# alenxav/bWGR

Measured on AMD Instinct MI355X. Metric: MCMC iter/sec (full marker sweep), higher is better.
Workload: dtype f32 scalars, fixed-point / f64 residual, int8 genotypes; 1 GPU; c4: synthetic n=10000 x p=1000000 int8, BayesB pi=0.99 (1.2% of the markers in the model at the last sweep), exact chain (blocked sweep, block=128, 40 slabs x 256 rows + 1 sequencer, the chain alone on the GPU: 80 streamers x 128 rows, engine generation 3, lag 12 blocks); n=10000, p=1000000, model=BayesB, df=5, chains=1

## Files before the change

bwgr_amd/csrc/sweep3.hip.h:

```cpp
#pragma once
#include "sweep2.hip.h"

namespace bwgr {

#ifdef BWGR_STAMPS
#define S3ST_DECL unsigned long long ph3[8] = {0, 0, 0, 0, 0, 0, 0, 0}, tl3 = __builtin_amdgcn_s_memtime()
#define S3ST(k, cond) do { if ((BWGR_STAMPS == 1 || (BWGR_STAMPS == 2 && ((k) == 0 || (k) == 1 || (k) == 4)) || (BWGR_STAMPS == 3 && ((k) == 0 || (k) == 4) && blockIdx.x == 0 && threadIdx.x == 0) || (BWGR_STAMPS == 4 && (k) <= 5 && blockIdx.x == 0 && threadIdx.x == 0)) && (cond)) { const unsigned long long t_ = __builtin_amdgcn_s_memtime(); ph3[k] += t_ - tl3; tl3 = t_; } } while (0)
#define S3ST_FLUSH(base, cond) do { if ((cond) && a.stamps) for (int k_ = 0; k_ < 8; ++k_) atomicAdd(&a.stamps[(base) + k_], ph3[k_]); } while (0)
#else
#define S3ST_DECL do { } while (0)
#define S3ST(k, cond) do { } while (0)
#define S3ST_FLUSH(base, cond) do { } while (0)
#endif

static constexpr int S3_MAXD = 16;
static constexpr int S3_LSTRIDE = 2 * SW_MAXM + 2;
static constexpr int S3_ND = 7;
static constexpr int S3_RING = S3_MAXD * SW_MAXM;
static constexpr int S3_GPD_BYTES = 16384;
static constexpr int S3_ROWSLOT = 1024;
static constexpr int S3_NRX = 8;
static constexpr int S3_OS = 12;
static constexpr int S3_NFW = 4;
static constexpr int S3_NFL = 8;
// ... 477 lines not shown
#undef S3_COMMIT1
#undef S3_TILE_COMMIT
}

template <int R3, int NTB, typename SH = S3ShapeAny>
__device__ __forceinline__ void s3_streamer_dma(const Sweep3Args &A) {
#ifdef BWGR_EXPERIMENTS
  const int SDBG = A.dbg;
#else
  constexpr int SDBG = 0;
#endif
  extern __shared__ __attribute__((aligned(16))) unsigned char smem[];
  const SweepArgs &a = A.a;
  const int tid = threadIdx.x, lane = tid & 63, wave = tid >> 6;
  const int m16 = lane & 15, grp = lane >> 4;
  const int w = s3_stream_index(A);
  const unsigned long long *lists_w = A.lists;
  const int m = s3_m<SH>(a), R = a.R, D = A.D;
  constexpr int Rp = R3 + 16;
  constexpr int CH = R3 / 16;
  constexpr int MPP = 1024 / R3;
  constexpr int NPC = SW_MAXM / MPP;
  static_assert(R3 == 128 || R3 == 256, "sixteen or thirty-two pieces");
  const int slab = w / A.sub, hsub = w - slab * A.sub;
  const int nb = a.blk_end - a.blk_begin;
  constexpr int NU = R3 >> 6;
  const int8_t *Xs = reinterpret_cast<const int8_t *>(a.X) + (size_t)slab * a.p * R + (size_t)hsub * R3;
  const int64_t row0 = (int64_t)slab * R + (int64_t)hsub * R3;
  uint32_t *abortw = a.xflags + (size_t)a.K * SW_FLAG_STRIDE;
  constexpr size_t tile_b = (size_t)SW_MAXM * R3;
  int8_t *tile0 = reinterpret_cast<int8_t *>(smem);
  size_t off = NTB * tile_b;
  const uint32_t tile_la = (uint32_t)__builtin_amdgcn_readfirstlane((int)(uint32_t)(uintptr_t)(__attribute__((address_space(3))) const unsigned char *)smem);
  int8_t *edig0 = reinterpret_cast<int8_t *>(smem + off); off += (size_t)2 * 16 * Rp;
  int8_t *ddig0 = reinterpret_cast<int8_t *>(smem + off); off += (size_t)2 * 16 * S2_DP;
  int *outu = reinterpret_cast<int *>(smem + off); off += (size_t)64 * S3_OS * 4 * 4;
  off += (size_t)8 * 32 * S3_OS * 4;
  uint32_t *ctl_s = reinterpret_cast<uint32_t *>(smem + off); off += 64;
  float *drej_s = reinterpret_cast<float *>(smem + off);
  const uint32_t drej_la = (uint32_t)__builtin_amdgcn_readfirstlane((int)(uint32_t)(uintptr_t)(__attribute__((address_space(3))) const unsigned char *)drej_s);
  const int sh = a.sc->e3_sh;
  const double S = s3_pow2(sh), invS = s3_pow2(-sh);
  auto blk_j0 = [&](int b) { return (a.blk_begin + b) * m; };
  auto blk_m = [&](int b) { return min(m, a.p - (a.blk_begin + b) * m); };

  for (int i = tid; i < (int)((2 * 16 * Rp + 2 * 16 * S2_DP) / 4); i += SW_THREADS) reinterpret_cast<uint32_t *>(edig0)[i] = 0u;
  if (tid < 16) ctl_s[tid] = 0u;
  long long e_own = 0;
  const bool upd = wave < NU;
  if (upd) e_own = __double2ll_rn(a.e[row0 + 64 * wave + lane] * S);

  static_assert(NU == 2, "waves 0-1 update, 2-5 dots, 6-7 DMA");
  constexpr int NDOT = 4, PPW = NPC / 2;
  static_assert(NU + NDOT == 6 && SW_THREADS - SW_MAXM == 64 * (NU + NDOT), "the DMA waves (role 2) are the last two: they digitise the rejected steps");
  constexpr int LPS = PPW + 2;
  const uint32_t lane_mk = (uint32_t)(lane / CH), lane_cr = (uint32_t)(lane % CH);
  const int j_lo = a.blk_begin * m, j_hi = min(a.p, a.blk_end * m);
  const int wvs = __builtin_amdgcn_readfirstlane(wave);
  auto drej_issue = [&](int t) {
    const unsigned char *src = reinterpret_cast<const unsigned char *>(a.ps.blocks[a.blk_begin + max(0, min(t, nb - 1))].drej);
    const uint32_t la = drej_la + (uint32_t)((max(t, 0) % NTB) * SW_MAXM * 4);
    s3_dma4s(src, (uint32_t)lane * 4u, la);
    s3_dma4s(src, 256u + (uint32_t)lane * 4u, la + 256u);
  };
  auto tile_issue = [&](int t) {
    if (wvs < 6) return;
    const int jb = blk_j0(min(t, nb - 1));
    const uint32_t la0 = tile_la + (uint32_t)__builtin_amdgcn_readfirstlane((int)((t % NTB) * (int)tile_b));
#pragma unroll
    for (int u = 0; u < PPW; ++u) {
      const int pc = (wvs - 6) + 2 * u;
      const int jl = MPP * pc + (int)lane_mk;
      const int jj = min(jb + jl, j_hi - 1);
      const uint32_t voff = (uint32_t)(jj - j_lo) * (uint32_t)R + ((lane_cr ^ ((uint32_t)jl & (uint32_t)(CH - 1))) * 16u);
      s3_dma16s(reinterpret_cast<const unsigned char *>(Xs + (size_t)j_lo * R), voff, la0 + (uint32_t)pc * 1024u);
    }
    drej_issue(t + 1);
  };

  auto fold_list = [&](int bs, unsigned long long pre, int e_first = 0) -> int {
    const int Bs = a.blk_begin + bs;
    const unsigned long long *L = lists_w + (size_t)Bs * S3_LSTRIDE;
    const int8_t *col = Xs + (size_t)(Bs * m) * R + 64 * wave + lane;
    const uint64_t t0 = wall_clock64();
    unsigned spins = 0;
    unsigned long long hv = __builtin_amdgcn_readfirstlane((uint32_t)pre) | ((unsigned long long)__builtin_amdgcn_readfirstlane((uint32_t)(pre >> 32)) << 32);
    while (!s3_epoch_is(hv, A.epoch)) {
      hv = ld_agent_raw64(L);
      hv = __builtin_amdgcn_readfirstlane((uint32_t)hv) | ((unsigned long long)__builtin_amdgcn_readfirstlane((uint32_t)(hv >> 32)) << 32);
      if (s3_epoch_is(hv, A.epoch)) break;
      if ((++spins & 63u) == 0u) {
        if (ld_agent_u32(abortw) != 0u) return 0;
        if (wall_clock64() - t0 > SW_TIMEOUT_TICKS) { st_agent_u32(abortw, 1u); return 0; }
      }
      __builtin_amdgcn_s_sleep(1);
    }
    const int cnt = (int)(uint32_t)hv;
    for (int c0 = 0; c0 < cnt; c0 += 31) {
      const int nw = min(62, 2 * (cnt - c0));
      unsigned long long wv = pre;
      bool have = (c0 == 0);
      for (;;) {
        const bool mine = lane >= 1 && lane <= nw;
        if (!have) wv = mine ? ld_agent_raw64(L + 2 * c0 + lane) : 0ull;
        if (__ballot(mine && !s3_epoch_is(wv, A.epoch)) == 0ull) break;
        have = false;
        if ((++spins & 63u) == 0u) {
          if (ld_agent_u32(abortw) != 0u) return 0;
          if (wall_clock64() - t0 > SW_TIMEOUT_TICKS) { st_agent_u32(abortw, 1u); return 0; }
        }
        __builtin_amdgcn_s_sleep(1);
      }
      const uint32_t wlo = (uint32_t)wv, whi = (uint32_t)(wv >> 32);
      for (int e0 = (c0 == 0) ? e_first : 0; e0 < nw / 2; e0 += 8) {
        int xb[8]; long long cq[8];
#pragma unroll
        for (int u = 0; u < 8; ++u) {
          const int ee = min(e0 + u, nw / 2 - 1);
          const uint32_t a0 = __builtin_amdgcn_readlane(wlo, 1 + 2 * ee), a1 = __builtin_amdgcn_readlane(whi, 1 + 2 * ee);
          const uint32_t b0 = __builtin_amdgcn_readlane(wlo, 2 + 2 * ee);
          const int k = (int)(a1 & 0xFFu);
          cq[u] = (e0 + u < nw / 2) ? (long long)(((unsigned long long)b0 << 32) | (unsigned long long)a0) : 0ll;
          xb[u] = upd ? (int)col[(size_t)k * R] : 0;
        }
#pragma unroll
        for (int u = 0; u < 8; ++u) e_own -= (long long)xb[u] * cq[u];
      }
    }
    return 1;
  };

  constexpr int NPRE = 4;
  int xp0 = 0, xp1 = 0, xp2 = 0, xp3 = 0;
  long long cp0 = 0, cp1 = 0, cp2 = 0, cp3 = 0;
  int np = -1;
#ifndef BWGR_WORDS2
#define BWGR_WORDS2 0
#endif
  unsigned long long lmid = 0ull, lw1 = 0ull;
#define S3_PAR(A0_, A1_) (*((!BWGR_WORDS2 || PP == 0) ? &(A0_) : &(A1_)))
  auto fold_prefetch = [&](int bs, auto par_c) {
    constexpr int PP = decltype(par_c)::value;
    const unsigned long long wv = S3_PAR(lmid, lw1);
    const unsigned long long hv = __builtin_amdgcn_readfirstlane((uint32_t)wv) | ((unsigned long long)__builtin_amdgcn_readfirstlane((uint32_t)(wv >> 32)) << 32);
    const int cnt = (int)(uint32_t)hv, nw = min(62, 2 * max(cnt, 0));
    const bool ok = bs >= 0 && s3_epoch_is(hv, A.epoch) && __ballot(lane >= 1 && lane <= nw && !s3_epoch_is(wv, A.epoch)) == 0ull;
    const int8_t *col = Xs + (size_t)((a.blk_begin + max(bs, 0)) * m) * R + 64 * wave + lane;
    const uint32_t wlo = (uint32_t)wv, whi = (uint32_t)(wv >> 32);
    const int ne = ok ? nw / 2 : 0;
#define S3_PRE1(U_, XP_, CP_) { \
      const int ee = min(U_, max(ne - 1, 0)); \
      const uint32_t a0 = __builtin_amdgcn_readlane(wlo, 1 + 2 * ee), a1 = __builtin_amdgcn_readlane(whi, 1 + 2 * ee), b0 = __builtin_amdgcn_readlane(wlo, 2 + 2 * ee); \
      CP_ = (U_ < ne) ? (long long)(((unsigned long long)b0 << 32) | (unsigned long long)a0) : 0ll; \
      XP_ = (int)col[(size_t)(ne > 0 ? (int)(a1 & 0xFFu) : 0) * R]; }
    S3_PRE1(0, xp0, cp0) S3_PRE1(1, xp1, cp1) S3_PRE1(2, xp2, cp2) S3_PRE1(3, xp3, cp3)
#undef S3_PRE1
    np = (bs < 0) ? 0 : (ok ? cnt : -1);
  };
  auto fold_pre = [&](int bs) -> int {
#ifdef BWGR_EXPERIMENTS
    if (w == 0 && tid == 0 && a.stamps && (SDBG & (1 << 21))) { atomicAdd(&a.stamps[203], 1ull); if (np < 0) atomicAdd(&a.stamps[202], 1ull); }
#endif
    if (np < 0) return fold_list(bs, 0ull);
    e_own -= (long long)xp0 * cp0 + (long long)xp1 * cp1 + (long long)xp2 * cp2 + (long long)xp3 * cp3;
    return (np > NPRE) ? fold_list(bs, 0ull, NPRE) : 1;
  };

  if (wvs >= 6) drej_issue(0);
  for (int t = 0; t < NTB - 1; ++t) tile_issue(t);
  if (wvs < NU) {
    lmid = ld_agent_raw64(lists_w + (size_t)(a.blk_begin + max(min(1, nb - 1) - D, 0)) * S3_LSTRIDE + lane);
    if (BWGR_WORDS2) lw1 = ld_agent_raw64(lists_w + (size_t)(a.blk_begin + max(min(2, nb - 1) - D, 0)) * S3_LSTRIDE + lane);
  }
  asm volatile("s_waitcnt vmcnt(0)" ::: "memory");
  __syncthreads();
  S3ST_DECL;
  [[maybe_unused]] const bool st_u = (w == 0 && tid == 0), st_d = (w == 0 && tid == 64 * NU);

  constexpr int WN = (NTB - 2) * LPS;
#define S3_DMA_BARRIER() do { if constexpr (DMA) asm volatile("s_waitcnt vmcnt(%0)" : : "n"(WN) : "memory"); asm volatile("s_waitcnt lgkmcnt(0)\n\ts_barrier" ::: "memory"); } while (0)
  auto step = [&](int b, auto par_c, auto role_c) -> bool {
    constexpr int PP = decltype(par_c)::value;
    constexpr int RL = decltype(role_c)::value;
    constexpr bool UPD = RL == 0, DMA = RL == 2;
    const int mB = blk_m(b), par = b & 1;
    S3ST(0, st_u || st_d);
    int8_t *tile = tile0 + (size_t)(b % NTB) * tile_b;
    int8_t *edig = edig0 + (size_t)par * 16 * Rp;
    int8_t *ddig = ddig0 + (size_t)par * 16 * S2_DP;
    if (b >= D && UPD && !(SDBG & 512)) { if (!fold_pre(b - D)) ctl_s[0] = 1u; }
#ifndef BWGR_FOLD_EARLY
#define BWGR_FOLD_EARLY 1
// ... 140 lines not shown
  const int tid = threadIdx.x, lane = tid & 63, wave = tid >> 6;
  static_assert(!SH::fixed || (sizeof(GT) == 2 && !CEN), "the fixed shape: 16-bit Gram entries, columns as stored");
  const int m = s3_m<SH>(a), nb = a.blk_end - a.blk_begin, D = A.D, pstride = s3_pstride<SH>(a);
  size_t off = 0;
  StageBuf *stage = reinterpret_cast<StageBuf *>(smem + off); off += 3 * sizeof(StageBuf);
  double *spec_s = reinterpret_cast<double *>(smem + off); off += (size_t)3 * 2 * SW_MAXM * sizeof(double);
  double *q_s = reinterpret_cast<double *>(smem + off); off += (size_t)2 * SW_MAXM * sizeof(double);
  double *far_s = reinterpret_cast<double *>(smem + off); off += (size_t)2 * S3_NFW * SW_MAXM * sizeof(double);
  float *state_s = reinterpret_cast<float *>(smem + off); off += (size_t)2 * 3 * SW_MAXM * sizeof(float);
  double *accC = reinterpret_cast<double *>(smem + off); off += (size_t)S3_RING * sizeof(double);
  float2 *accS = reinterpret_cast<float2 *>(smem + off); off += (size_t)S3_RING * sizeof(float2);
  int *accK = reinterpret_cast<int *>(smem + off); off += (size_t)S3_RING * sizeof(int);
  unsigned char *rowf_s = smem + off; off += (size_t)2 * S3_NFW * S3_NFL * SW_MAXM * sizeof(GT);
  constexpr bool G16 = (sizeof(GT) == 2);
#ifndef BWGR_GPD3
#define BWGR_GPD3 1
#endif
  constexpr bool GPD = G16 && (BWGR_GPD3 != 0);
  unsigned char *gpd_s = smem + off; if (G16) off += (size_t)3 * S3_GPD_BYTES;
  unsigned char *rowx_s = smem + off; if (G16) off += (size_t)S3_NRX * S3_ROWSLOT;
  unsigned char *qraw_s = smem + off; off += (size_t)3 * S3_QRAW_BYTES;
  unsigned char *touch_s = smem + off; off += 256;
  int *ctrl_s = reinterpret_cast<int *>(smem + off);
  int *pos_s = ctrl_s + 8;
  const unsigned char **gx_s = reinterpret_cast<const unsigned char **>(ctrl_s + 40);
  S3ST_DECL;
  const GT *gp_all = reinterpret_cast<const GT *>(A.gp);
  const float Cc = a.sc->C, odds = a.sc->odds, one_minus_pi = 1.0f - a.sc->pi, Sb = a.sc->Sb;
  const int sh = a.sc->e3_sh;
  const double S = s3_pow2(sh), invS = s3_pow2(-sh);
  uint32_t *abortw = a.xflags + (size_t)a.K * SW_FLAG_STRIDE;
  auto blk_m = [&](int b) { return min(m, a.p - (a.blk_begin + b) * m); };
  auto prow = [&](int k) { return k * (m - 1) - k * (k - 1) / 2; };
  constexpr int NCH = (int)(sizeof(StageBuf) / 16);
  static_assert(NCH + 128 == 512, "four 16-byte chunks for each lane of the two staging waves");

  constexpr int S3_STG_PIECES = 4 + (GPD ? 8 : 0);
  const uint32_t stage_la = (uint32_t)__builtin_amdgcn_readfirstlane((int)(uint32_t)(uintptr_t)(__attribute__((address_space(3))) const unsigned char *)stage);
  const uint32_t spec_la = (uint32_t)__builtin_amdgcn_readfirstlane((int)(uint32_t)(uintptr_t)(__attribute__((address_space(3))) const unsigned char *)spec_s);
  static_assert(sizeof(StageBuf) == 6 * 1024, "six 1 KiB pieces of constants");
  auto stage_issue = [&](int c, int part = -1) {
    const int blk = a.blk_begin + min(c, nb - 1), slot = c % 3, wv2 = __builtin_amdgcn_readfirstlane(wave) - 2;
    const unsigned char *stb = reinterpret_cast<const unsigned char *>(a.ps.blocks + blk);
    const unsigned char *spb = reinterpret_cast<const unsigned char *>(a.ps.spec + blk);
    const uint32_t lo16 = (uint32_t)lane * 16u;
    if (part <= 0) {
#pragma unroll
    for (int u = 0; u < 3; ++u) { const int pc = wv2 + 2 * u; s3_dma16s(stb, (uint32_t)pc * 1024u + lo16, stage_la + (uint32_t)slot * (uint32_t)sizeof(StageBuf) + (uint32_t)pc * 1024u); }
    s3_dma16s(spb, (uint32_t)wv2 * 2048u + lo16, spec_la + (uint32_t)slot * 2048u + (uint32_t)wv2 * 1024u);
    }
    if constexpr (GPD) {
      const int gpbytes = pstride * 2;
      const unsigned char *src = reinterpret_cast<const unsigned char *>(gp_all + (size_t)blk * pstride);
      const uint32_t gla = (uint32_t)__builtin_amdgcn_readfirstlane((int)(uint32_t)(uintptr_t)(__attribute__((address_space(3))) const unsigned char *)gpd_s) + (uint32_t)slot * (uint32_t)S3_GPD_BYTES;
      if (part < 0 || part == 1) {
#pragma unroll
      for (int u = 0; u < 4; ++u) { const int pc = wv2 + 2 * u; s3_dma16s(src, (uint32_t)min(pc * 1024 + lane * 16, gpbytes - 16), gla + (uint32_t)pc * 1024u); }
      }
      if (part < 0 || part == 2) {
#pragma unroll
      for (int u = 4; u < 8; ++u) { const int pc = wv2 + 2 * u; s3_dma16s(src, (uint32_t)min(pc * 1024 + lane * 16, gpbytes - 16), gla + (uint32_t)pc * 1024u); }
      }
    }
  };
#define S3_STG_WAIT() asm volatile("s_waitcnt vmcnt(%0)" : : "n"(S3_STG_PIECES) : "memory")
  const uint32_t qraw_la = (uint32_t)__builtin_amdgcn_readfirstlane((int)(uint32_t)(uintptr_t)(__attribute__((address_space(3))) const unsigned char *)qraw_s);
  const double qweight = (SH::fixed || A.qsplit) ? 4294967296.0 : 16777216.0;
  auto poll_request = [&](int c) {
    const unsigned char *g = reinterpret_cast<const unsigned char *>(A.qsum + (size_t)(a.blk_begin + min(c, nb - 1)) * SW_MAXM * 2);
    const uint32_t la = qraw_la + (uint32_t)((c % 3) * S3_QRAW_BYTES);
    s3_dma16s_sc1(g, (uint32_t)lane * 16u, la);
    s3_dma16s_sc1(g, 1024u + (uint32_t)lane * 16u, la + 1024u);
  };
  auto poll_q = [&](int c) -> int {
    const int mBc = blk_m(c);
    const unsigned long long *g = A.qsum + (size_t)(a.blk_begin + c) * SW_MAXM * 2;
    const unsigned long long need = (unsigned long long)A.K3;
    const bool n0 = lane < mBc, n1 = 64 + lane < mBc;
    asm volatile("s_waitcnt vmcnt(2)" ::: "memory");
    const ulonglong2 v0 = reinterpret_cast<const ulonglong2 *>(qraw_s + (size_t)(c % 3) * S3_QRAW_BYTES)[lane];
    const ulonglong2 v1 = reinterpret_cast<const ulonglong2 *>(qraw_s + (size_t)(c % 3) * S3_QRAW_BYTES)[64 + lane];
    unsigned long long l0 = n0 ? v0.x : need, h0 = n0 ? v0.y : need, l1 = n1 ? v1.x : need, h1 = n1 ? v1.y : need;
    if (__builtin_expect(!(SDBG & 8) && __ballot(!((l0 & 0xFFull) == need && (h0 & 0xFFull) == need && (l1 & 0xFFull) == need && (h1 & 0xFFull) == need)) != 0ull, 0)) {
      const uint64_t t0 = wall_clock64();
      unsigned spins = 0;
#ifdef BWGR_EXPERIMENTS
      if (lane == 0 && a.stamps && (SDBG & (1 << 21))) atomicAdd(&a.stamps[200], 1ull);
#endif
      for (;;) {
        if ((l0 & 0xFFull) == need && (h0 & 0xFFull) == need && (l1 & 0xFFull) == need && (h1 & 0xFFull) == need) break;
        if (SDBG & 8) break;
#ifdef BWGR_EXPERIMENTS
        if (lane == 0 && a.stamps && (SDBG & (1 << 21))) atomicAdd(&a.stamps[201], 1ull);
#endif
        if ((++spins & 63u) == 0u) {
          if (ld_agent_u32(abortw) != 0u) return 0;
          if (wall_clock64() - t0 > SW_TIMEOUT_TICKS) { st_agent_u32(abortw, 1u); return 0; }
        }
        __builtin_amdgcn_s_sleep(1);
        if (n0) { l0 = ld_agent_raw64(g + 2 * lane); h0 = ld_agent_raw64(g + 2 * lane + 1); }
        if (n1) { l1 = ld_agent_raw64(g + 2 * (64 + lane)); h1 = ld_agent_raw64(g + 2 * (64 + lane) + 1); }
      }
    }
    double *qd = q_s + (size_t)(c & 1) * SW_MAXM;
    qd[lane] = n0 ? fma((double)((long long)h0 >> 8), qweight, (double)((long long)l0 >> 8)) * invS : 0.0;
    qd[64 + lane] = n1 ? fma((double)((long long)h1 >> 8), qweight, (double)((long long)l1 >> 8)) * invS : 0.0;
    poll_request(c + 2);
    return 1;
  };
  constexpr int ring = S3_RING;
  static_assert((S3_RING & (S3_RING - 1)) == 0, "ring positions wrap with a mask");
  constexpr int NFL = S3_NFL;
  constexpr int NFW = S3_NFW;
  constexpr int ROWB = SW_MAXM * (int)sizeof(GT);
  constexpr int NPC = ROWB / 256;
  int f_p0 = 0, f_cnt = 0, f_n = 0;
  const uint32_t rowf_la = (uint32_t)__builtin_amdgcn_readfirstlane((int)(uint32_t)(uintptr_t)(__attribute__((address_space(3))) const unsigned char *)rowf_s);
  const int rowbytes = m * (int)sizeof(GT);
  auto far_src = [&](int c, int sl) -> const unsigned char * {
    const int kb = accK[sl];
    const int d = c - (kb >> 8);
    return gx_s[d - 1] + ((size_t)(a.blk_begin + c) * m * m + (size_t)(kb & 0xFF) * m) * sizeof(GT);
  };
  auto far_add = [&](const uint32_t *row, double cf, double &s0, double &s1) {
    if constexpr (sizeof(GT) == 2) { const uint32_t v = row[lane]; s0 = fma((double)(v & 0xFFFFu), cf, s0); s1 = fma((double)(v >> 16), cf, s1); }
    else { s0 = fma((double)(int)row[lane], cf, s0); s1 = fma((double)(int)row[64 + lane], cf, s1); }
  };
  unsigned long long f_ptr = 0ull;
  double f_cf = 0.0;
#ifndef BWGR_FARTOUCH
#define BWGR_FARTOUCH 1
#endif
  auto far_touch = [&](int c) {
    if (!G16 || !BWGR_FARTOUCH || c < 2 || D < 4 || (SDBG & 32)) return;
    const int s_blk = c - 2;
    const int p0 = pos_s[s_blk & 31], cnt = (pos_s[(s_blk + 1) & 31] - p0) & (ring - 1);
    const int q = lane & 31, d = 3 + (q >> 1);
    for (int e0 = 0; e0 < cnt; e0 += 2) {
      const int e = e0 + (lane >> 5);
      if (e < cnt && d <= D - 1 && s_blk + d < nb && (q & 1) * 128 < rowbytes) {
        const int k = accK[(p0 + e) & (ring - 1)] & 0xFF;
        s3_dma4(gx_s[d - 1] + ((size_t)(a.blk_begin + s_blk + d) * m * m + (size_t)k * m) * sizeof(GT) + (size_t)(q & 1) * 128, touch_s);
      }
    }
  };
  int fp_a = 0, fp_b = 0, fp_kb = 0; double fp_cf = 0.0; bool fp_on = false;
  auto far_plan_a = [&](int c) {
    fp_on = !(c < 3 || D < 4 || c >= nb || (SDBG & 32));
    fp_a = pos_s[max(c - D + 1, 0) & 31]; fp_b = pos_s[(max(c, 2) - 2) & 31];
  };
  auto far_plan_b = [&](int c, int hw) {
    f_p0 = fp_a;
    f_cnt = fp_on ? ((fp_b - fp_a) & (ring - 1)) : 0;
    f_n = (f_cnt > hw) ? min(NFL, (f_cnt - hw + NFW - 1) / NFW) : 0;
    const int sl = (f_p0 + hw + NFW * min(lane, max(f_n - 1, 0))) & (ring - 1);
    fp_kb = accK[sl]; fp_cf = accC[sl];
  };
  auto far_plan_c = [&](int c) {
    const int d = min(max(c - (fp_kb >> 8), 1), S3_MAXD);
    const unsigned char *src = gx_s[d - 1] + ((size_t)(a.blk_begin + c) * m * m + (size_t)(fp_kb & 0xFF) * m) * sizeof(GT);
    f_ptr = (f_n > 0) ? (unsigned long long)src : 0ull;
    f_cf = (lane < f_n) ? fp_cf : 0.0;
  };
  auto far_plan = [&](int c, int hw) { far_plan_a(c); far_plan_b(c, hw); far_plan_c(c); };
  auto far_request = [&](int c, int hw) {
    const uint32_t dst_la = (uint32_t)__builtin_amdgcn_readfirstlane((int)(rowf_la + (uint32_t)(((c & 1) * NFW + hw) * NFL) * (uint32_t)ROWB));
    for (int n = 0; n < f_n; ++n) {
      const unsigned char *src = reinterpret_cast<const unsigned char *>(
          (unsigned long long)(uint32_t)__builtin_amdgcn_readlane((int)(uint32_t)f_ptr, n) |
          ((unsigned long long)(uint32_t)__builtin_amdgcn_readlane((int)(uint32_t)(f_ptr >> 32), n) << 32));
#pragma unroll
      for (int pc = 0; pc < NPC; ++pc) s3_dma4s(src, (uint32_t)min(lane * 4 + 256 * pc, rowbytes - 4), dst_la + (uint32_t)(n * ROWB + 256 * pc));
    }
  };
  auto far_consume = [&](int c, int hw, int f_p0, int f_cnt, int f_n, double f_cf) {
    double s0 = 0.0, s1 = 0.0, t0 = 0.0, t1 = 0.0;
    const unsigned char *src = rowf_s + (size_t)(((c & 1) * NFW + hw) * NFL) * ROWB;
    int n = 0;
    if constexpr (sizeof(GT) == 2) {
      for (; n + 4 <= f_n; n += 4) {
// ... 46 lines not shown
  double sum_d = 0.0, sum_b2 = 0.0;
  double chn0 = 1.0, chn1 = 1.0;
  auto chi_request = [&](int c) {
    const StageBuf &sb = a.ps.blocks[a.blk_begin + max(0, min(c, nb - 1))];
    chn0 = sb.chi[lane]; chn1 = sb.chi[64 + lane];
  };
  auto finish_block = [&](int c) {
    const int blk = a.blk_begin + c, j0c = blk * m, mBc = blk_m(c);
    const float *sp = state_s + (size_t)(c & 1) * 2 * SW_MAXM;
    const bool vbv = (a.flags & SWF_VB_VEC) != 0 && !A.skip_vb;
    const double ch0 = chn0, ch1 = chn1;
    if (vbv) chi_request(c + 1);
#pragma unroll
    for (int h = 0; h < 2; ++h) {
      const int t = lane + 64 * h;
      if (t < mBc) {
        const float bn = sp[t], dn = sp[SW_MAXM + t];
        a.b[j0c + t] = bn;
        a.d[j0c + t] = dn;
        if (vbv) a.vb[j0c + t] = (float)((double)(Sb + bn * bn) / (h ? ch1 : ch0));
        sum_d += (double)dn;
        sum_b2 = fma((double)bn, (double)bn, sum_b2);
      }
    }
    const int p0 = pos_s[c & 31], cnt = (pos_s[(c + 1) & 31] - p0) & (ring - 1);
    unsigned long long *L = A.lists + (size_t)blk * S3_LSTRIDE;
    for (int w0 = 0; w0 < 1 + 2 * cnt; w0 += 64) {
      const int wi = w0 + lane;
      if (wi < 1 + 2 * cnt) {
        unsigned long long v;
        if (wi == 0) v = s3_hdr(A.epoch, cnt);
        else {
          const int sl = (p0 + ((wi - 1) >> 1)) & (ring - 1);
          const float2 st2 = accS[sl];
          const long long cq = (long long)rint((double)st2.x * S) - (long long)rint((double)st2.y * S);
          v = ((wi - 1) & 1) ? (((unsigned long long)A.epoch << 40) | (0xEEull << 32) | ((unsigned long long)cq >> 32))
                             : (((unsigned long long)A.epoch << 40) | ((unsigned long long)(uint32_t)(accK[sl] & 0xFF) << 32) | ((unsigned long long)cq & 0xFFFFFFFFull));
        }
        st_agent_raw64(L + wi, v);
      }
    }
  };
#ifndef BWGR_ROLEBAR
#define BWGR_ROLEBAR 1
#endif
#define S3_ROLE_BARRIER() do { if (BWGR_ROLEBAR) asm volatile("s_waitcnt lgkmcnt(0)\n\ts_barrier" ::: "memory"); } while (0)
  const int wvu = __builtin_amdgcn_readfirstlane(wave);

  if (tid < 40) ctrl_s[tid] = (tid == 0) ? 1 : 0;
  if (tid >= 64 && tid < 64 + S3_MAXD) gx_s[tid - 64] = reinterpret_cast<const unsigned char *>(A.gx[tid - 64]);
  __syncthreads();
  if (wave == 1) { poll_request(0); poll_request(1); if (!poll_q(0)) ctrl_s[0] = 0; }
  else if (wave == 2 || wave == 3) { stage_issue(0); stage_issue(1); S3_STG_WAIT(); far_consume(0, wave, 0, 0, 0, 0.0); far_plan(1, wave); far_request(1, wave); }
  else if (wave >= 5 && wave <= 6) { far_consume(0, wave - 5, 0, 0, 0, 0.0); far_plan(1, wave - 5); far_request(1, wave - 5); }
  else if (wave == 7) { for (int c = 0; c < PF; ++c) touch(c); if ((a.flags & SWF_VB_VEC) && !A.skip_vb) chi_request(0); }
  __syncthreads();
  if (ctrl_s[0] == 0) { if (tid == 0) a.sc->error = 1u; asm volatile("s_waitcnt vmcnt(0)" ::: "memory"); return; }
  [[maybe_unused]] const bool sq0 = (tid == 0), sq1 = (tid == 64), sq2 = (tid == 128), sq4 = (tid == 320), sq3 = (tid == 192), sq6 = (tid == 384), sq7 = (tid == 448);
#define S3_BLOCK_END(SQ_, ABORT_) \
    if (!BWGR_ROLEBAR) asm volatile("s_waitcnt lgkmcnt(0)\n\ts_barrier" ::: "memory"); \
    S3ST(4, SQ_); \
    if (ctrl_s[0] == 0) { asm volatile("s_waitcnt vmcnt(0)" ::: "memory"); ABORT_; }
  auto helper_loop = [&](auto &&phase, const bool sq) -> bool {
    for (int b = 0; b < nb; ++b) {
      S3ST(0, sq);
      if (b + 1 < nb) { phase(b + 1); S3ST(1, sq); }
      else S3_ROLE_BARRIER();
      S3_BLOCK_END(sq, return false)
    }
    return true;
  };
  if (wvu == 0) {
    const int tabp0 = 2 * (lane * (m - 1) - lane * (lane - 1) / 2 - lane - 1);
    const int tabp1 = 2 * ((64 + lane) * (m - 1) - (64 + lane) * (63 + lane) / 2 - (64 + lane) - 1);
    const uint32_t rolane16 = (uint32_t)min(lane * 16, 2 * rowbytes - 16);
    const unsigned char *gpd_lane = gpd_s + 2 * lane;
    int gpd_off = 0;
    const uint32_t rowx_la = (uint32_t)__builtin_amdgcn_readfirstlane((int)(uint32_t)(uintptr_t)(__attribute__((address_space(3))) const unsigned char *)rowx_s);
    const bool altb2 = (a.flags & SWF_ALT_B2) != 0;
    if (wave == 0 && !(SDBG & 1)) __builtin_amdgcn_s_setprio(3);
    double rnext0 = 0.0, rnext1 = 0.0, rnxt20 = 0.0, rnxt21 = 0.0;
    int pend_n = 0, pend_p = 0;
    bool pend_u1 = false, pend_u2 = false;
    const double ninv = a.ninv;
    const double cen_u0 = CEN ? a.sc->cen_u0 : 0.0;
    double cenU = cen_u0;
    const GT *gx0_w0 = reinterpret_cast<const GT *>(A.gx[0]) + (size_t)a.blk_begin * m * m, *gx1_w0 = reinterpret_cast<const GT *>(A.gx[1]) + (size_t)a.blk_begin * m * m;
    const unsigned char *g12_w0 = A.gx12 + (size_t)a.blk_begin * m * 2 * rowbytes;
    if (!(SDBG & 1)) __builtin_amdgcn_s_setprio(3);
    auto block = [&](int b) {
      const int mB = blk_m(b), blk = a.blk_begin + b;
      const bool have_next = (b + 1 < nb);
      const StageBuf &st = stage[b % 3];
      const double *sps = spec_s + (size_t)(b % 3) * 2 * SW_MAXM;
      const double *qd = q_s + (size_t)(b & 1) * SW_MAXM;
      const double *fd = far_s + (size_t)(b & 1) * S3_NFW * SW_MAXM;
      const int pos0 = pos_s[b & 31];
      const GT *gp = gp_all + (size_t)blk * pstride;
      const bool use1 = have_next && D >= 2;
      const GT *g1 = (G16 || use1) ? gx0_w0 + (size_t)(b + 1) * (uint32_t)(m * m) : gp;
      const bool use2 = (b + 2 < nb) && D >= 3;
      const GT *g2 = (G16 || use2) ? gx1_w0 + (size_t)(b + 2) * (uint32_t)(m * m) : gp;
      const unsigned char *g12b = g12_w0 + (size_t)b * (uint32_t)(m * 2 * rowbytes);
      const int l0 = lane, l1 = 64 + lane;
      const int l1c = min(l1, m - 1), l0c = min(l0, m - 1);
      const float b0a = st.b0[l0], b0b = st.b0[l1], b2a = st.b2[l0], b2b = st.b2[l1], dra = st.drej[l0], drb = st.drej[l1];
      const float taa = st.tacc[l0], tab = st.tacc[l1], tra = st.trej[l0], trb = st.trej[l1];
      const double xba = (double)st.xxb0[l0], xbb = (double)st.xxb0[l1];
      const double rda = st.rden[l0], rdb = st.rden[l1], sza = st.sdz1[l0], szb = st.sdz1[l1];
      double gja = sps[SW_MAXM + l0], gjb = sps[SW_MAXM + l1];
      double r0 = (qd[l0] - sps[l0]) - ((fd[l0] + fd[SW_MAXM + l0]) + (fd[2 * SW_MAXM + l0] + fd[3 * SW_MAXM + l0]));
      double r1 = (qd[l1] - sps[l1]) - ((fd[l1] + fd[SW_MAXM + l1]) + (fd[2 * SW_MAXM + l1] + fd[3 * SW_MAXM + l1]));
      if constexpr (G16) {
        if (pend_n > 0) {
          asm volatile("s_waitcnt vmcnt(0) lgkmcnt(0)" ::: "memory");
          for (int i_ = 0; i_ < pend_n; ++i_) {
            const double cf_ = accC[(pend_p + i_) & (ring - 1)];
            const uint16_t *rw1_ = reinterpret_cast<const uint16_t *>(rowx_s + (size_t)i_ * S3_ROWSLOT);
            const uint16_t *rw2_ = rw1_ + m;
            const uint32_t x1a_ = rw1_[l0c], x1b_ = rw1_[l1c], x2a_ = rw2_[l0c], x2b_ = rw2_[l1c];
            const double c1_ = pend_u1 ? cf_ : 0.0, c2_ = pend_u2 ? cf_ : 0.0;
            rnext0 = fma(-(double)x1a_, c1_, rnext0); rnext1 = fma(-(double)x1b_, c1_, rnext1);
            rnxt20 = fma(-(double)x2a_, c2_, rnxt20); rnxt21 = fma(-(double)x2b_, c2_, rnxt21);
          }
          pend_n = 0;
        }
      }
      r0 += rnext0; r1 += rnext1;
      int csa = 0, csb = 0;
      double sA = 0.0, sB = 0.0;
      if constexpr (CEN) {
        csa = __double2hiint(gja); csb = __double2hiint(gjb);
        sA = (double)csa; sB = (double)csb;
        gja = (double)(uint32_t)__double2loint(gja) - sA * sA * ninv; gjb = (double)(uint32_t)__double2loint(gjb) - sB * sB * ninv;
        r0 = fma(sA, cenU, r0); r1 = fma(sB, cenU, r1);
      }
      const double D2a = (double)((altb2 ? b2a : 0.0f) - b0a), D2b = (double)((altb2 ? b2b : 0.0f) - b0b);
      const double D2sa = D2a * D2a, D2sb = D2b * D2b;
      rnext0 = rnxt20; rnext1 = rnxt21; rnxt20 = 0.0; rnxt21 = 0.0;
      S3ST(1, sq0);
      unsigned long long am0 = 0ull, am1 = 0ull;
      int nacc = 0, nslot = 0, napp = 0;
#define S3_EVAL(R_, XB_, RD_, SZ_, B0_, D2_, D2S_, GJ_, TA_, TR_, MKOFF_, D1F_, ACC_) { \
        const float b1_ = (float)fma((R_) + (XB_), (RD_), (SZ_)); \
        D1F_ = b1_ - (B0_); \
        const double D1_ = (double)D1F_; \
        const double diffd_ = fma((GJ_), (D2S_) - D1_ * D1_, (2.0 * (R_)) * (D1_ - (D2_)));    \
        const float x_ = Cc * (float)diffd_; \
         \
        const unsigned long long ma_ = __ballot(x_ < (TA_)); \
        const unsigned long long mu_ = ~(ma_ | __ballot(x_ > (TR_)));    \
        ACC_ = ma_; \
        if (__builtin_expect(mu_ != 0ull, 0)) { \
          const bool ex_ = lane_accept_exact(diffd_, a.marker0 + (uint32_t)(blk * m + (MKOFF_) + lane), a.flags, Cc, odds, one_minus_pi, a.rng, a.iter); \
          ACC_ |= __ballot(ex_) & mu_; \
        } }
#define S3_APPLY_ROWS() { \
        asm volatile("s_waitcnt vmcnt(0) lgkmcnt(0)" ::: "memory"); \
         \
        for (int i_ = 0; i_ < nslot; ++i_) { \
          const double cf_ = accC[(pos0 + napp + i_) & (ring - 1)]; \
          const uint16_t *rw1_ = reinterpret_cast<const uint16_t *>(rowx_s + (size_t)i_ * S3_ROWSLOT); \
          const uint16_t *rw2_ = rw1_ + m; \
          const uint32_t x1a_ = rw1_[l0c], x1b_ = rw1_[l1c], x2a_ = rw2_[l0c], x2b_ = rw2_[l1c]; \
          const double c1_ = use1 ? cf_ : 0.0, c2_ = use2 ? cf_ : 0.0; \
          rnext0 = fma(-(double)x1a_, c1_, rnext0); rnext1 = fma(-(double)x1b_, c1_, rnext1); \
          rnxt20 = fma(-(double)x2a_, c2_, rnxt20); rnxt21 = fma(-(double)x2b_, c2_, rnxt21); \
        } \
        napp += nslot; nslot = 0; }
#define S3_INCLUDE(KOFF_, D1F_, DR_) { \
        const int k_ = (KOFF_) + js; \
        GT ga_ = (GT)1, gb_ = (GT)1; \
        if constexpr (G16) { \
          if (!(SDBG & 64)) { \
          if constexpr (GPD) { \
            const unsigned char *gpl_ = gpd_lane + gpd_off + __builtin_amdgcn_readlane((KOFF_) ? tabp1 : tabp0, js); \
            ga_ = *reinterpret_cast<const GT *>(gpl_); gb_ = *reinterpret_cast<const GT *>(gpl_ + 128);    \
          } else { \
            const int pr_ = prow(k_); \
            ga_ = gp[min(pr_ + max(l0 - k_ - 1, 0), pstride - 1)]; gb_ = gp[min(pr_ + max(l1c - k_ - 1, 0), pstride - 1)]; \
          } \
          if (__builtin_expect(nslot == S3_NRX, 0)) S3_APPLY_ROWS()    \
          if (use1) s3_dma16s(g12b, rolane16 + (uint32_t)(k_ * 2 * rowbytes), rowx_la + (uint32_t)nslot * S3_ROWSLOT); \
          ++nslot; } \
        } else if (!(SDBG & 64)) {    \
          const int pr_ = prow(k_); \
          ga_ = gp[min(pr_ + max(l0 - k_ - 1, 0), pstride - 1)]; gb_ = gp[min(pr_ + max(l1c - k_ - 1, 0), pstride - 1)];    \
        } \
        const float dacc_ = readlane_f32(D1F_, js), drj_ = readlane_f32(DR_, js); \
        const double corr_ = (double)dacc_ - (double)drj_; \
        if (lane == 0) { const int sl_ = (pos0 + nacc) & (ring - 1); accK[sl_] = k_ | (b << 8); accC[sl_] = corr_; accS[sl_] = make_float2(dacc_, drj_); } \
        ++nacc; \
        if constexpr (CEN) { \
          const double xk_ = (double)__builtin_amdgcn_readlane((KOFF_) ? csb : csa, js) * ninv;    \
          cenU = fma(xk_, corr_, cenU); \
          r0 = fma(-((l0 > k_) ? ((double)ga_ - sA * xk_) : 0.0), corr_, r0); \
          r1 = fma(-((l1 > k_ && l1 < m) ? ((double)gb_ - sB * xk_) : 0.0), corr_, r1); \
        } else { \
        r0 = fma(-(double)((l0 > k_) ? ga_ : (GT)0), corr_, r0); \
        r1 = fma(-(double)((l1 > k_ && l1 < m) ? gb_ : (GT)0), corr_, r1); \
        } \
        if constexpr (!G16) { if (!(SDBG & 64)) { \
          const GT *row_ = g1 + (use1 ? (size_t)k_ * m : (size_t)0);    \
          const GT xa_ = row_[use1 ? min(l0, m - 1) : 0], xb_ = row_[use1 ? l1c : 0]; \
          const GT *row2_ = g2 + (use2 ? (size_t)k_ * m : (size_t)0); \
          const GT ya_ = row2_[use2 ? min(l0, m - 1) : 0], yb_ = row2_[use2 ? l1c : 0]; \
          if (use1) { rnext0 = fma(-(double)xa_, corr_, rnext0); rnext1 = fma(-(double)xb_, corr_, rnext1); } \
          if (use2) { rnxt20 = fma(-(double)ya_, corr_, rnxt20); rnxt21 = fma(-(double)yb_, corr_, rnxt21); } } } }
      if (!(SDBG & 128)) {
        const int cnt0 = min(64, mB);
        unsigned long long live0 = (cnt0 >= 64) ? ~0ull : ((1ull << cnt0) - 1ull);
        for (;;) {
          float d1f; unsigned long long acc;
          S3_EVAL(r0, xba, rda, sza, b0a, D2a, D2sa, gja, taa, tra, 0, d1f, acc)
          const unsigned long long bal = acc & live0;
          if (bal == 0ull) break;
          const int js = (int)__builtin_ctzll(bal);
          live0 &= (~1ull << js);
          am0 |= 1ull << js;
          S3_INCLUDE(0, d1f, dra)
        }
      }
      if (mB > 64 && (!(SDBG & 128))) {
        const int cnt1 = mB - 64;
        unsigned long long live1 = (cnt1 >= 64) ? ~0ull : ((1ull << cnt1) - 1ull);
        for (;;) {
          float d1f; unsigned long long acc;
          S3_EVAL(r1, xbb, rdb, szb, b0b, D2b, D2sb, gjb, tab, trb, 64, d1f, acc)
          const unsigned long long bal = acc & live1;
          if (bal == 0ull) break;
          const int js = (int)__builtin_ctzll(bal);
          live1 &= (~1ull << js);
          am1 |= 1ull << js;
          S3_INCLUDE(64, d1f, drb)
        }
      }
#undef S3_EVAL
#undef S3_INCLUDE
      S3ST(5, sq0);
      if constexpr (G16) { pend_n = nslot; pend_p = pos0 + napp; pend_u1 = use1; pend_u2 = use2; }
#undef S3_APPLY_ROWS
      S3ST(2, sq0);
      {
        float *sp = state_s + (size_t)(b & 1) * 2 * SW_MAXM;
        const float b1a = (float)fma(r0 + xba, rda, sza), b1b = (float)fma(r1 + xbb, rdb, szb);
        const bool ia = ((am0 >> lane) & 1ull) != 0ull, ib = ((am1 >> lane) & 1ull) != 0ull;
        sp[l0] = ia ? b1a : b2a; sp[l1] = ib ? b1b : b2b;
        sp[SW_MAXM + l0] = ia ? 1.0f : 0.0f; sp[SW_MAXM + l1] = ib ? 1.0f : 0.0f;
      }
      if (lane == 0) pos_s[(b + 1) & 31] = (pos0 + nacc) & (ring - 1);
      S3ST(3, sq0);
      gpd_off = (gpd_off == 2 * S3_GPD_BYTES) ? 0 : gpd_off + S3_GPD_BYTES;
      S3_ROLE_BARRIER();
    };
    for (int b = 0; b < nb; ++b) {
      S3ST(0, sq0);
      if (!(SDBG & 16384)) block(b);
      else S3_ROLE_BARRIER();
      S3_BLOCK_END(sq0, if (tid == 0) a.sc->error = 1u; return)
    }
    S3ST_FLUSH(16, sq0);
    if constexpr (CEN) { if (tid == 0) a.sc->cen_c = cenU - cen_u0; }
  } else if (wvu == 1) {
    if (!helper_loop([&](int c) { if (!(SDBG & 32768)) { if (!poll_q(c)) ctrl_s[0] = 0; } S3ST(2, tid == 64); S3_ROLE_BARRIER(); }, sq1)) return;
    S3ST_FLUSH(24, sq1);
    asm volatile("s_waitcnt vmcnt(0)" ::: "memory");
  } else if (wvu <= 3) {
    if (!helper_loop([&](int c) {
      if (!(SDBG & 8192)) {
        const int o_p0 = f_p0, o_cnt = f_cnt, o_n = f_n; const double o_cf = f_cf;
        far_plan_a(c + 1);
        stage_issue(c + 1, 0);
        far_plan_b(c + 1, wave);
        stage_issue(c + 1, 1);
        far_plan_c(c + 1);
        stage_issue(c + 1, 2);
        S3_STG_WAIT();
        far_consume(c, wave, o_p0, o_cnt, o_n, o_cf);
        far_request(c + 1, wave);
      }
      S3ST(2, tid == 128 || tid == 192); S3_ROLE_BARRIER(); }, sq2 || sq3)) return;
    S3ST_FLUSH(32, sq2); S3ST_FLUSH(48, sq3);
    asm volatile("s_waitcnt vmcnt(0)" ::: "memory");
  } else if (wvu == 4) {
    if (!helper_loop([&](int c) { far_touch(c); S3_ROLE_BARRIER(); }, false)) return;
    asm volatile("s_waitcnt vmcnt(0)" ::: "memory");
  } else if (wvu <= 6) {
    if (!helper_loop([&](int c) {
      const int o_p0 = f_p0, o_cnt = f_cnt, o_n = f_n; const double o_cf = f_cf;
      far_plan(c + 1, wave - 5);
      asm volatile("s_waitcnt vmcnt(0) lgkmcnt(0)" ::: "memory");
      S3ST(5, tid == 320);
      far_consume(c, wave - 5, o_p0, o_cnt, o_n, o_cf);
      S3ST(6, tid == 320);
      far_request(c + 1, wave - 5);
      S3ST(7, tid == 320);
      S3ST(2, tid == 384);
      S3_ROLE_BARRIER(); }, sq4 || sq6)) return;
    S3ST_FLUSH(40, sq4); S3ST_FLUSH(56, sq6);
  } else {
    if (!helper_loop([&](int c) { if (c >= 2 && !(SDBG & 4096)) finish_block(c - 2); touch(c + PF); S3ST(2, tid == 448); S3_ROLE_BARRIER(); }, sq7)) return;
    S3ST_FLUSH(64, sq7);
    if (nb >= 2) finish_block(nb - 2);
    finish_block(nb - 1);
#pragma unroll
    for (int o = 32; o > 0; o >>= 1) { sum_d += __shfl_down(sum_d, o, 64); sum_b2 += __shfl_down(sum_b2, o, 64); }
    if (lane == 0) { a.sc->sum_d += sum_d; a.sc->sum_b2 += sum_b2; }
  }
#undef S3_BLOCK_END
}

template <typename GT, bool ROWS, typename SH = S3ShapeAny>
__device__ __forceinline__ void s3_prefetcher(const Sweep3Args &A) {
  const SweepArgs &a = A.a;
  const int tid = threadIdx.x, nb = a.blk_end - a.blk_begin;
  constexpr int AHEAD = 16, NPB = 4;
  uint32_t *abortw = a.xflags + (size_t)a.K * SW_FLAG_STRIDE;
  const size_t gpbytes = (size_t)s3_pstride<SH>(a) * sizeof(GT);
  uint32_t sink = 0u;
  const size_t o = (size_t)tid * 128;
  for (int c0 = 0; c0 < nb; c0 += NPB) {
    const int clast = min(c0 + NPB, nb) - 1;
    if (clast >= AHEAD) {
      const unsigned long long *L = A.lists + (size_t)(a.blk_begin + clast - AHEAD) * S3_LSTRIDE;
      const uint64_t t0 = wall_clock64();
      unsigned spins = 0;
      for (;;) {
        if (s3_epoch_is(ld_agent_raw64(L), A.epoch)) break;
        if ((++spins & 63u) == 0u && (ld_agent_u32(abortw) != 0u || wall_clock64() - t0 > SW_TIMEOUT_TICKS)) return;
        __builtin_amdgcn_s_sleep(4);
      }
    }
    uint32_t v[NPB][3];
    const size_t g12bytes = (size_t)s3_m<SH>(a) * 2 * s3_m<SH>(a) * sizeof(GT);
#pragma unroll
    for (int u = 0; u < NPB; ++u) {
      const int blk = a.blk_begin + min(c0 + u, nb - 1);
      if (ROWS) {
        v[u][0] = *reinterpret_cast<const uint32_t *>(A.gx12 + (size_t)blk * g12bytes + min(o, g12bytes - 4));
        v[u][1] = 0u; v[u][2] = 0u;
      } else {
        const unsigned char *gpb = reinterpret_cast<const unsigned char *>(A.gp) + (size_t)blk * gpbytes;
        const unsigned char *stb = reinterpret_cast<const unsigned char *>(a.ps.blocks + blk);
        const unsigned char *spb = reinterpret_cast<const unsigned char *>(a.ps.spec + blk);
        v[u][0] = *reinterpret_cast<const uint32_t *>(stb + min(o, sizeof(StageBuf) - 4));
        v[u][1] = *reinterpret_cast<const uint32_t *>(spb + min(o, sizeof(SpecBuf) - 4));
        v[u][2] = *reinterpret_cast<const uint32_t *>(gpb + min(o, gpbytes - 4));
      }
    }
#pragma unroll
    for (int u = 0; u < NPB; ++u) sink += v[u][0] + v[u][1] + v[u][2];
  }
  if (sink == 0x9E3779B9u && a.stamps) a.stamps[255] = sink;
}

template <typename GT, bool CEN = false>
__global__ __launch_bounds__(SW_THREADS) void k_sweep3(const Sweep3Args A) {
  if (!(A.a.sc->inc_rate < A.a.gate3)) return;
  if ((int)blockIdx.x == A.pf) { s3_prefetcher<GT, false>(A); return; }
  if ((int)blockIdx.x == A.pf2) { s3_prefetcher<GT, true>(A); return; }
  if (blockIdx.x == 0) { if (!(A.dbg & 1024)) s3_sequencer<GT, CEN>(A); }
  else if ((A.a.flags & SWF_DEBUG_WITHHOLD) && blockIdx.x == 1 && A.pf != 1) return;
  else if (A.dbg & 2048) return;
  else if ((A.dbg & (1 << 22)) && !(A.dbg & (1 << 23)) && A.R3 == 128) s3_streamer_dma<128, 4>(A);
  else if ((A.dbg & (1 << 23)) && A.R3 == 128) s3_streamer_dma<128, 3>(A);
  else s3_streamer(A);
}

__global__ __launch_bounds__(SW_THREADS) void k_sweep3f(const Sweep3Args A) {
  if (!(A.a.sc->inc_rate < A.a.gate3)) return;
  if ((int)blockIdx.x == A.pf) { s3_prefetcher<uint16_t, false, S3Shape128>(A); return; }
  if ((int)blockIdx.x == A.pf2) { s3_prefetcher<uint16_t, true, S3Shape128>(A); return; }
#ifdef BWGR_EXPERIMENTS
  if (blockIdx.x == 0 ? (A.dbg & 1024) != 0 : (A.dbg & 2048) != 0) return;
#endif
  if (blockIdx.x == 0) s3_sequencer<uint16_t, false, S3Shape128>(A);
  else s3_streamer_dma<128, 4, S3Shape128>(A);
}

}
```

Baseline: 107.6 iter/s.

## Restructure prefetcher blocks with a progress-polling wave and multi-wave async DMA touches

The prefetcher blocks change shape. One wave now polls block-list publication, looking several blocks ahead, and posts its progress to LDS. The remaining waves split the blocks among themselves and touch every 8 KiB of each block's stage, spec, gp or gx12 data using async global-to-LDS loads, where before each thread did a single scalar read per block. Spin loops now read the wall clock only once the first 64 spins have passed, which moves a clock read off the fast path, and experiment-only wait counters are added. The change is meant to warm the cache for whole blocks with more loads in flight, at the cost of more memory traffic and extra LDS use.

```diff
diff --git a/bwgr_amd/csrc/sweep3.hip.h b/bwgr_amd/csrc/sweep3.hip.h
--- a/bwgr_amd/csrc/sweep3.hip.h
+++ b/bwgr_amd/csrc/sweep3.hip.h
@@ -583,7 +583,7 @@
     const int Bs = a.blk_begin + bs;
     const unsigned long long *L = lists_w + (size_t)Bs * S3_LSTRIDE;
     const int8_t *col = Xs + (size_t)(Bs * m) * R + 64 * wave + lane;
-    const uint64_t t0 = wall_clock64();
+    uint64_t t0 = 0;
     unsigned spins = 0;
     unsigned long long hv = __builtin_amdgcn_readfirstlane((uint32_t)pre) | ((unsigned long long)__builtin_amdgcn_readfirstlane((uint32_t)(pre >> 32)) << 32);
     while (!s3_epoch_is(hv, A.epoch)) {
@@ -592,7 +592,9 @@
       if (s3_epoch_is(hv, A.epoch)) break;
       if ((++spins & 63u) == 0u) {
         if (ld_agent_u32(abortw) != 0u) return 0;
-        if (wall_clock64() - t0 > SW_TIMEOUT_TICKS) { st_agent_u32(abortw, 1u); return 0; }
+        const uint64_t now = wall_clock64();
+        if (spins == 64u) t0 = now;
+        else if (now - t0 > SW_TIMEOUT_TICKS) { st_agent_u32(abortw, 1u); return 0; }
       }
       __builtin_amdgcn_s_sleep(1);
     }
@@ -608,7 +610,9 @@
         have = false;
         if ((++spins & 63u) == 0u) {
           if (ld_agent_u32(abortw) != 0u) return 0;
-          if (wall_clock64() - t0 > SW_TIMEOUT_TICKS) { st_agent_u32(abortw, 1u); return 0; }
+          const uint64_t now = wall_clock64();
+          if (spins == 64u) t0 = now;
+          else if (now - t0 > SW_TIMEOUT_TICKS) { st_agent_u32(abortw, 1u); return 0; }
         }
         __builtin_amdgcn_s_sleep(1);
       }
@@ -915,7 +919,7 @@
     const ulonglong2 v1 = reinterpret_cast<const ulonglong2 *>(qraw_s + (size_t)(c % 3) * S3_QRAW_BYTES)[64 + lane];
     unsigned long long l0 = n0 ? v0.x : need, h0 = n0 ? v0.y : need, l1 = n1 ? v1.x : need, h1 = n1 ? v1.y : need;
     if (__builtin_expect(!(SDBG & 8) && __ballot(!((l0 & 0xFFull) == need && (h0 & 0xFFull) == need && (l1 & 0xFFull) == need && (h1 & 0xFFull) == need)) != 0ull, 0)) {
-      const uint64_t t0 = wall_clock64();
+      uint64_t t0 = 0;
       unsigned spins = 0;
 #ifdef BWGR_EXPERIMENTS
       if (lane == 0 && a.stamps && (SDBG & (1 << 21))) atomicAdd(&a.stamps[200], 1ull);
@@ -928,7 +932,9 @@
 #endif
         if ((++spins & 63u) == 0u) {
           if (ld_agent_u32(abortw) != 0u) return 0;
-          if (wall_clock64() - t0 > SW_TIMEOUT_TICKS) { st_agent_u32(abortw, 1u); return 0; }
+          const uint64_t now = wall_clock64();
+          if (spins == 64u) t0 = now;
+          else if (now - t0 > SW_TIMEOUT_TICKS) { st_agent_u32(abortw, 1u); return 0; }
         }
         __builtin_amdgcn_s_sleep(1);
         if (n0) { l0 = ld_agent_raw64(g + 2 * lane); h0 = ld_agent_raw64(g + 2 * lane + 1); }
@@ -1141,6 +1147,9 @@
     double rnext0 = 0.0, rnext1 = 0.0, rnxt20 = 0.0, rnxt21 = 0.0;
     int pend_n = 0, pend_p = 0;
     bool pend_u1 = false, pend_u2 = false;
+#ifdef BWGR_EXPERIMENTS
+    unsigned long long w0_wait = 0ull, w0_nwait = 0ull;
+#endif
     const double ninv = a.ninv;
     const double cen_u0 = CEN ? a.sc->cen_u0 : 0.0;
     double cenU = cen_u0;
@@ -1172,7 +1181,13 @@
       double r1 = (qd[l1] - sps[l1]) - ((fd[l1] + fd[SW_MAXM + l1]) + (fd[2 * SW_MAXM + l1] + fd[3 * SW_MAXM + l1]));
       if constexpr (G16) {
         if (pend_n > 0) {
+#ifdef BWGR_EXPERIMENTS
+          const unsigned long long tw_ = (SDBG & (1 << 21)) ? __builtin_amdgcn_s_memtime() : 0ull;
+#endif
           asm volatile("s_waitcnt vmcnt(0) lgkmcnt(0)" ::: "memory");
+#ifdef BWGR_EXPERIMENTS
+          if (SDBG & (1 << 21)) { w0_wait += __builtin_amdgcn_s_memtime() - tw_; ++w0_nwait; }
+#endif
           for (int i_ = 0; i_ < pend_n; ++i_) {
             const double cf_ = accC[(pend_p + i_) & (ring - 1)];
             const uint16_t *rw1_ = reinterpret_cast<const uint16_t *>(rowx_s + (size_t)i_ * S3_ROWSLOT);
@@ -1319,12 +1334,18 @@
       S3_BLOCK_END(sq0, if (tid == 0) a.sc->error = 1u; return)
     }
     S3ST_FLUSH(16, sq0);
+#ifdef BWGR_EXPERIMENTS
+    if (sq0 && a.stamps && (SDBG & (1 << 21))) { atomicAdd(&a.stamps[211], w0_wait); atomicAdd(&a.stamps[212], w0_nwait); }
+#endif
     if constexpr (CEN) { if (tid == 0) a.sc->cen_c = cenU - cen_u0; }
   } else if (wvu == 1) {
     if (!helper_loop([&](int c) { if (!(SDBG & 32768)) { if (!poll_q(c)) ctrl_s[0] = 0; } S3ST(2, tid == 64); S3_ROLE_BARRIER(); }, sq1)) return;
     S3ST_FLUSH(24, sq1);
     asm volatile("s_waitcnt vmcnt(0)" ::: "memory");
   } else if (wvu <= 3) {
+#ifdef BWGR_EXPERIMENTS
+    unsigned long long stg_wait = 0ull;
+#endif
     if (!helper_loop([&](int c) {
       if (!(SDBG & 8192)) {
         const int o_p0 = f_p0, o_cnt = f_cnt, o_n = f_n; const double o_cf = f_cf;
@@ -1334,12 +1355,21 @@
         stage_issue(c + 1, 1);
         far_plan_c(c + 1);
         stage_issue(c + 1, 2);
+#ifdef BWGR_EXPERIMENTS
+        const unsigned long long tw_ = (SDBG & (1 << 21)) ? __builtin_amdgcn_s_memtime() : 0ull;
+#endif
         S3_STG_WAIT();
+#ifdef BWGR_EXPERIMENTS
+        if (SDBG & (1 << 21)) stg_wait += __builtin_amdgcn_s_memtime() - tw_;
+#endif
         far_consume(c, wave, o_p0, o_cnt, o_n, o_cf);
         far_request(c + 1, wave);
       }
       S3ST(2, tid == 128 || tid == 192); S3_ROLE_BARRIER(); }, sq2 || sq3)) return;
     S3ST_FLUSH(32, sq2); S3ST_FLUSH(48, sq3);
+#ifdef BWGR_EXPERIMENTS
+    if ((sq2 || sq3) && a.stamps && (SDBG & (1 << 21))) { atomicAdd(&a.stamps[210], stg_wait); if (sq2) atomicAdd(&a.stamps[213], (unsigned long long)nb); }
+#endif
     asm volatile("s_waitcnt vmcnt(0)" ::: "memory");
   } else if (wvu == 4) {
     if (!helper_loop([&](int c) { far_touch(c); S3_ROLE_BARRIER(); }, false)) return;
@@ -1369,48 +1399,94 @@
 #undef S3_BLOCK_END
 }
 
+#ifndef BWGR_PF_AHEAD
+#define BWGR_PF_AHEAD 16
+#endif
+#ifndef BWGR_PF_NPB
+#define BWGR_PF_NPB 4
+#endif
+static constexpr int S3_PF_STOP = -2;
+static constexpr int S3_PF_LOOK = 8;
 template <typename GT, bool ROWS, typename SH = S3ShapeAny>
 __device__ __forceinline__ void s3_prefetcher(const Sweep3Args &A) {
+  extern __shared__ __attribute__((aligned(16))) unsigned char smem[];
   const SweepArgs &a = A.a;
-  const int tid = threadIdx.x, nb = a.blk_end - a.blk_begin;
-  constexpr int AHEAD = 16, NPB = 4;
-  uint32_t *abortw = a.xflags + (size_t)a.K * SW_FLAG_STRIDE;
+  const int tid = threadIdx.x, lane = tid & 63, nb = a.blk_end - a.blk_begin;
+  const int wvs = __builtin_amdgcn_readfirstlane(tid >> 6);
+  constexpr int AHEAD = BWGR_PF_AHEAD, NPB = BWGR_PF_NPB, NTW = SW_THREADS / 64 - 1;
+  constexpr int NGP = (SW_MAXM * (SW_MAXM - 1) / 2 * (int)sizeof(GT) + 8191) / 8192;
+  constexpr int RPB = ROWS ? SW_MAXM * 2 * SW_MAXM * (int)sizeof(GT) / 8192 : 2 + NGP;
+  static_assert(sizeof(StageBuf) <= 8192 && sizeof(SpecBuf) <= 8192, "one request each");
+  constexpr int GRP = (NPB * RPB <= 28) ? NPB : (4 * RPB <= 28 && NPB % 4 == 0) ? 4 : (2 * RPB <= 28 && NPB % 2 == 0) ? 2 : 1;
+  static_assert(NPB % GRP == 0 && 2 * GRP * RPB <= 56, "two groups of requests in flight per wave");
+  volatile __attribute__((address_space(3))) int *prog_s = (volatile __attribute__((address_space(3))) int *)(smem + 256 * (SW_THREADS / 64));
+  if (tid == 0) *prog_s = -1;
+  __syncthreads();
+  if (wvs == 0) {
+    uint32_t *abortw = a.xflags + (size_t)a.K * SW_FLAG_STRIDE;
+    const int target = nb - 1 - AHEAD;
+    int seen = -1;
+    unsigned spins = 0;
+    uint64_t t0 = 0;
+    bool stop = false;
+    while (seen < target && !stop) {
+      const bool pub = s3_epoch_is(ld_agent_raw64(A.lists + (size_t)(a.blk_begin + min(seen + 1 + min(lane, S3_PF_LOOK - 1), nb - 1)) * S3_LSTRIDE), A.epoch);
+      const unsigned long long bal = __ballot(pub);
+      if (bal != 0ull) {
+        seen = min(seen + 64 - (int)__builtin_clzll(bal), nb - 1);
+        *prog_s = seen;
+        spins = 0;
+      } else {
+        if ((++spins & 63u) == 0u) {
+          const uint64_t now = wall_clock64();
+          if (spins == 64u) t0 = now;
+          stop = ld_agent_u32(abortw) != 0u || now - t0 > SW_TIMEOUT_TICKS;
+        }
+        __builtin_amdgcn_s_sleep(4);
+      }
+    }
+    if (stop) *prog_s = S3_PF_STOP;
+    return;
+  }
   const size_t gpbytes = (size_t)s3_pstride<SH>(a) * sizeof(GT);
-  uint32_t sink = 0u;
-  const size_t o = (size_t)tid * 128;
-  for (int c0 = 0; c0 < nb; c0 += NPB) {
-    const int clast = min(c0 + NPB, nb) - 1;
+  const size_t g12bytes = (size_t)s3_m<SH>(a) * 2 * s3_m<SH>(a) * sizeof(GT);
+  const uint32_t pad_la = (uint32_t)__builtin_amdgcn_readfirstlane((int)(uint32_t)(uintptr_t)(__attribute__((address_space(3))) const unsigned char *)(smem + 256 * wvs));
+  const uint32_t o = (uint32_t)lane * 128u;
+  for (int t = wvs - 1; t * NPB < nb; t += NTW) {
+    const int c0 = t * NPB, clast = min(c0 + NPB, nb) - 1;
     if (clast >= AHEAD) {
-      const unsigned long long *L = A.lists + (size_t)(a.blk_begin + clast - AHEAD) * S3_LSTRIDE;
-      const uint64_t t0 = wall_clock64();
-      unsigned spins = 0;
-      for (;;) {
-        if (s3_epoch_is(ld_agent_raw64(L), A.epoch)) break;
-        if ((++spins & 63u) == 0u && (ld_agent_u32(abortw) != 0u || wall_clock64() - t0 > SW_TIMEOUT_TICKS)) return;
-        __builtin_amdgcn_s_sleep(4);
-      }
-    }
-    uint32_t v[NPB][3];
-    const size_t g12bytes = (size_t)s3_m<SH>(a) * 2 * s3_m<SH>(a) * sizeof(GT);
-#pragma unroll
+      int pr = __builtin_amdgcn_readfirstlane(*prog_s);
+#ifdef BWGR_EXPERIMENTS
+      const bool first_ = pr + AHEAD >= clast;
+#endif
+      while (pr != S3_PF_STOP && pr + AHEAD < clast) { __builtin_amdgcn_s_sleep(2); pr = __builtin_amdgcn_readfirstlane(*prog_s); }
+      if (pr == S3_PF_STOP) break;
+#ifdef BWGR_EXPERIMENTS
+      if (lane == 0 && a.stamps && (A.dbg & (1 << 21))) {
+        atomicAdd(&a.stamps[ROWS ? 207 : 204], 1ull);
+        if (first_) atomicAdd(&a.stamps[ROWS ? 208 : 205], 1ull);
+        atomicAdd(&a.stamps[ROWS ? 209 : 206], (unsigned long long)(c0 - pr));
+      }
+#endif
+    }
+#pragma nounroll
     for (int u = 0; u < NPB; ++u) {
+      if ((u & (GRP - 1)) == 0) asm volatile("s_waitcnt vmcnt(%0)" : : "n"(GRP * RPB) : "memory");
       const int blk = a.blk_begin + min(c0 + u, nb - 1);
-      if (ROWS) {
-        v[u][0] = *reinterpret_cast<const uint32_t *>(A.gx12 + (size_t)blk * g12bytes + min(o, g12bytes - 4));
-        v[u][1] = 0u; v[u][2] = 0u;
+      if constexpr (ROWS) {
+        const unsigned char *src = A.gx12 + (size_t)blk * g12bytes;
+#pragma nounroll
+        for (int r = 0; r < RPB; ++r) s3_dma4s(src, min(o + 8192u * r, (uint32_t)g12bytes - 4u), pad_la);
       } else {
+        s3_dma4s(reinterpret_cast<const unsigned char *>(a.ps.blocks + blk), min(o, (uint32_t)sizeof(StageBuf) - 4u), pad_la);
+        s3_dma4s(reinterpret_cast<const unsigned char *>(a.ps.spec + blk), min(o, (uint32_t)sizeof(SpecBuf) - 4u), pad_la);
         const unsigned char *gpb = reinterpret_cast<const unsigned char *>(A.gp) + (size_t)blk * gpbytes;
-        const unsigned char *stb = reinterpret_cast<const unsigned char *>(a.ps.blocks + blk);
-        const unsigned char *spb = reinterpret_cast<const unsigned char *>(a.ps.spec + blk);
-        v[u][0] = *reinterpret_cast<const uint32_t *>(stb + min(o, sizeof(StageBuf) - 4));
-        v[u][1] = *reinterpret_cast<const uint32_t *>(spb + min(o, sizeof(SpecBuf) - 4));
-        v[u][2] = *reinterpret_cast<const uint32_t *>(gpb + min(o, gpbytes - 4));
-      }
-    }
-#pragma unroll
-    for (int u = 0; u < NPB; ++u) sink += v[u][0] + v[u][1] + v[u][2];
+#pragma nounroll
+        for (int r = 0; r < NGP; ++r) s3_dma4s(gpb, min(o + 8192u * r, (uint32_t)gpbytes - 4u), pad_la);
+      }
+    }
   }
-  if (sink == 0x9E3779B9u && a.stamps) a.stamps[255] = sink;
+  asm volatile("s_waitcnt vmcnt(0)" ::: "memory");
 }
 
 template <typename GT, bool CEN = false>
```

Measured after the change: 106.6 iter/s. About the same (-0.9%).
